# openMVG/openMVG

Measured on NVIDIA B200. Metric: BA LM-iters/sec, higher is better.
Workload: dtype f64

## Files before the change

openmvg_b200/csrc/ba.cu:

```cuda
#include "ba_kernels.cuh"
#include <cub/device/device_radix_sort.cuh>

#include <algorithm>
#include <cmath>
#include <cstring>
#include <limits>
#include <memory>
#include <chrono>
#include <vector>

using namespace omvg;
using namespace omvg::ba;

namespace {

enum Slot { S_COST = 0, S_MODEL, S_STEP2_PT, S_STEP2_POSE, S_STEP2_INTR, S_X2_PT, S_X2_POSE, S_X2_INTR,
            S_GMAX_PT, S_GMAX_CAM, S_GMAX_INTR, S_PCG_IT, S_PCG_RES, S_PCG_B, S_CAND_COST, S_COUNT = 16 };

int model_nparams(int m) {
  switch (m) { case 1: return 3; case 2: return 4; case 3: return 6; case 4: return 8; case 5: return 7; case OMVG_CAMERA_SPHERICAL: return 0; default: return -1; }
}
int model_ndata(int m) { return m == OMVG_CAMERA_SPHERICAL ? 2 : model_nparams(m); }

template <typename T> struct DevBuf {
// ... 17 lines not shown
  int ni8 = 0, nred = 0, words = 0, nnzb = 0, eval_blocks = 0, eval_grid = 0, kiu = KI, gj_grid = 0, ics_chunks = 64;
  std::vector<int> perm;
  DevBuf<int> d_perm;
  std::vector<int> h_intr_model;
  DevBuf<double> pose[2], intr[2], pt[2], pose0, intr0, pt0;
  DevBuf<int> intr_model, obs_pose, obs_intr, obs_pt, pt_start, cam_start, cam_obs;
  DevBuf<double> obs_xy;
  DevBuf<double> r, Jp, Jc, Ji, camR[2], camdR, camrec[2];
  DevBuf<double> sc_pt, sc_cam, sc_intr, diag_pt, diag_cam, diag_intr, lmD_pt, lmD_cam, lmD_intr, g_cam, g_intr;
  DevBuf<double> EtE, Etb, EtFi, FtF, FiFi, Einv, step_pt, step_red;
  DevBuf<unsigned char> pt_single;
  DevBuf<unsigned> bitmap, intr_mask; DevBuf<int> wprefix, rowptr, cols;
  DevBuf<double> Scc, Sci, Sii, rhs, Minv_c, Minv_i, work_i;
  DevBuf<double> z, res, pvec, w, zeta, pcg_part;
  DevBuf<double> gW, bX, bR, bP, bW, bZ, pcg2_part;
  DevBuf<int> agg_of, agg_start, agg_cams, brow, nb_start, nb_list; DevBuf<unsigned short> blk_lcol; int nb_max = 0;
  DevBuf<double> cE, cT, cCv, cYv, cCv2, cAW, bP2; int ng = 0, agg_maxsize = 0;
  DevBuf<double> dA, dT;
  DevBuf<double> part, part2, part3, icol_part, scal;
  DevBuf<int> fail;
  DevBuf<unsigned long long> pcg_tim;
  DevBuf<double> corner_rep;
  DevBuf<double> GE;
  DevBuf<double> obs_w; DevBuf<unsigned char> obs_flags, pt_fixed; DevBuf<unsigned> pt_mask;
  DevBuf<unsigned char> pt_gcp, pt_removed, pt_now; DevBuf<unsigned> rej_bits; DevBuf<unsigned long long> rej_cnt;
  bool reject_ready = false;
  int n_slow = 0;
  bool has_ext = false; int npri = 0; double prior_huber_a = 0; DevBuf<int> prior_pose; DevBuf<double> prior_center, prior_weight, rP, JP;
  double *h_scal = nullptr;
  cudaEvent_t ev0 = nullptr, ev1 = nullptr, evj0 = nullptr, evj1 = nullptr;
  long long launches = 0;
};

namespace {

#define LAUNCH_CHECK() OMVG_CUDA(cudaGetLastError())

struct PhaseTimer {
  bool on = getenv("OMVG_BA_TIMING") != nullptr; const char *what;
  std::chrono::steady_clock::time_point t0 = std::chrono::steady_clock::now();
  explicit PhaseTimer(const char *w) : what(w) {}
  void lap(const char *name) { if (!on) return; const auto t1 = std::chrono::steady_clock::now(); fprintf(stderr, "[omvg_ba timing] %s/%s %.3f ms\n", what, name, std::chrono::duration<double, std::milli>(t1 - t0).count()); t0 = t1; }
};

int validate(const omvg_ba_problem *P) {
  if (!P) return fail(OMVG_E_ARG, "null problem");
// ... 224 lines not shown
  { std::vector<int> nb_start(ng + 1, 0), nb_list; std::vector<unsigned short> lcol(c->nnzb, 0); std::vector<int> mark(c->nc, -1);
    c->nb_max = 0;
    for (int g = 0; g < ng; ++g) {
      const int first = (int)nb_list.size();
      for (int t = agg_start[g]; t < agg_start[g + 1]; ++t) { const int a = agg_cams[t];
        for (int e = hp[a]; e < hp[a + 1]; ++e) { const int b = hcols[e]; if (mark[b] < first) { mark[b] = (int)nb_list.size(); nb_list.push_back(b); } lcol[e] = (unsigned short)std::min(65535, mark[b] - first); } }
      nb_start[g + 1] = (int)nb_list.size(); c->nb_max = std::max(c->nb_max, nb_start[g + 1] - first);
    }
    if ((rc = upload(c->nb_start, nb_start.data(), ng + 1, c->stream))) return rc;
    if ((rc = upload(c->nb_list, nb_list.data(), nb_list.size(), c->stream))) return rc;
    if ((rc = upload(c->blk_lcol, lcol.data(), lcol.size(), c->stream))) return rc;
    OMVG_CUDA(cudaStreamSynchronize(c->stream)); }
  const size_t nco_max = (size_t)ng * MAXW;
  if ((rc = c->cE.alloc(nco_max * nco_max))) return rc;
  if ((rc = c->cT.alloc(3 * (size_t)GJ_B * nco_max))) return rc;
  if ((rc = c->cCv.alloc((size_t)MAXRHS * nco_max))) return rc;
  if ((rc = c->cYv.alloc((size_t)MAXRHS * nco_max))) return rc;
  if ((rc = c->cCv2.alloc((size_t)MAXRHS * nco_max + 1)) || (rc = c->cAW.alloc((size_t)MAXRHS * nco_max + 1))) return rc;
  if ((rc = c->bP2.alloc((size_t)MAXRHS * 6 * c->nc))) return rc;
  OMVG_CUDA(cudaStreamSynchronize(c->stream));
  return c->Scc.alloc((size_t)c->nnzb * 36);
}

}

extern "C" {

void omvg_trim_cache(void) {
  omvg::pool_trim();
  ResPool &rp = res_pool(); std::lock_guard<std::mutex> g(rp.mu);
  int cur = 0; cudaGetDevice(&cur);
  for (int d = 0; d < 16; ++d) { if (rp.free_[d].empty()) continue; cudaSetDevice(d);
    for (CtxRes &r : rp.free_[d]) { cudaFreeHost(r.h_scal); for (cudaEvent_t e : r.ev) cudaEventDestroy(e); cudaStreamDestroy(r.stream); cudaStreamDestroy(r.stream2); }
    rp.free_[d].clear(); }
  cudaSetDevice(cur);
}

void omvg_ba_default_options(omvg_ba_options *o) {
  if (!o) return;
  std::memset(o, 0, sizeof *o);
  o->intrinsics_opt = 14; o->extrinsics_opt = 6; o->structure_opt = 1; o->use_loss = 1; o->huber_a = 16.0;
  o->max_num_iterations = 50; o->max_consecutive_invalid_steps = 5;
  o->function_tolerance = 1e-6; o->gradient_tolerance = 1e-10; o->parameter_tolerance = 1e-8;
  o->initial_radius = 1e4; o->max_radius = 1e16; o->min_radius = 1e-32; o->min_relative_decrease = 1e-3;
  o->min_lm_diagonal = 1e-6; o->max_lm_diagonal = 1e32;
  o->pcg_tolerance = 1e-8; o->pcg_max_iterations = 2000; o->verbose = 0;
// ... 89 lines not shown
  for (int w = 0; w < 2; ++w) { AL(c->pose[w], 6 * c->nc); AL(c->intr[w], c->ni8); AL(c->pt[w], 3 * (size_t)c->np); AL(c->camR[w], 9 * c->nc); AL(c->camrec[w], (size_t)CAMREC * c->nc); }
  AL(c->camdR, 27 * c->nc);
  AL(c->r, 2 * no); AL(c->Jp, 6 * no); AL(c->Jc, 12 * no); AL(c->Ji, 2 * KI * no);
  AL(c->sc_pt, 3 * (size_t)c->np); AL(c->sc_cam, 6 * c->nc); AL(c->sc_intr, c->ni8);
  AL(c->diag_pt, 3 * (size_t)c->np); AL(c->diag_cam, 6 * c->nc); AL(c->diag_intr, c->ni8);
  AL(c->lmD_pt, 3 * (size_t)c->np); AL(c->lmD_cam, 6 * c->nc); AL(c->lmD_intr, c->ni8); AL(c->g_cam, 6 * c->nc); AL(c->g_intr, c->ni8);
  AL(c->EtFi, 3 * KI * (size_t)c->np); AL(c->FtF, 36 * (size_t)c->nc); AL(c->FiFi, 64 * (size_t)c->ni);
  AL(c->EtE, 6 * (size_t)c->np); AL(c->Etb, 3 * (size_t)c->np); AL(c->Einv, 9 * (size_t)c->np); AL(c->step_pt, 3 * (size_t)c->np); AL(c->step_red, c->nred);
  AL(c->intr_mask, c->ni);
  AL(c->Sci, (size_t)c->ni8 * 6 * c->nc); AL(c->Sii, (size_t)c->ni8 * c->ni8); AL(c->rhs, c->nred); AL(c->Minv_c, 36 * (size_t)c->nc); AL(c->Minv_i, (size_t)c->ni * KI * KI);
  AL(c->work_i, (size_t)c->ni8 * c->ni8 + c->ni8);
  AL(c->gW, (size_t)MAXW * 6 * c->nc);
  AL(c->bX, (size_t)MAXRHS * 6 * c->nc); AL(c->bR, (size_t)MAXRHS * 6 * c->nc); AL(c->bP, (size_t)MAXRHS * 6 * c->nc); AL(c->bW, (size_t)MAXRHS * 6 * c->nc); AL(c->bZ, (size_t)MAXRHS * 6 * c->nc);
  AL(c->pcg2_part, (size_t)c->n_sms * PCG2_V);
  AL(c->z, c->nred); AL(c->res, c->nred); AL(c->pvec, c->nred); AL(c->w, c->nred); AL(c->zeta, c->nred); AL(c->pcg_part, 3 * (size_t)c->n_sms * 2);
  if (c->npri) { AL(c->rP, 3 * c->npri); AL(c->JP, 18 * c->npri); }
  AL(c->part, std::max(c->eval_blocks, 1024) + 2); AL(c->part2, 1024); AL(c->part3, 1024); c->ics_chunks = (int)std::max<long long>(1, std::min<long long>(4ll * c->n_sms / std::max(1, c->ni), (c->no + 2047) / 2048));
  AL(c->icol_part, (size_t)c->ni * c->ics_chunks * ICS_W); AL(c->scal, S_COUNT); AL(c->fail, 1);
#undef AL
  OMVG_CUDA(cudaMemsetAsync(c->scal.p, 0, S_COUNT * sizeof(double), s));
  tm.lap("allocations");
  if ((rc = build_structure(c))) return rc;
  tm.lap("structure");
  OMVG_CUDA(cudaStreamWaitEvent(s, c->ev_up, 0));
  setup_gather_xy_kernel<<<(unsigned)((no + 255) / 256), 256, 0, s>>>(c->d_perm.p, reinterpret_cast<const double2 *>(raw_xy.p), raw_w.p, raw_fl.p, no,
                                                                  reinterpret_cast<double2 *>(c->obs_xy.p), c->obs_w.p, c->obs_flags.p); LAUNCH_CHECK();
  c->launches++;
  if ((rc = omvg_ba_reset(c))) return rc;
  OMVG_CUDA(cudaStreamSynchronize(s));
  guard.release();
  *out = c; return OMVG_OK;
}

int omvg_ba_reset(omvg_ba_ctx *c) {
  if (!c) return fail(OMVG_E_ARG, "null ctx");
  OMVG_CUDA(cudaSetDevice(c->device));
  OMVG_CUDA(cudaMemcpyAsync(c->pose[0].p, c->pose0.p, 6 * c->nc * sizeof(double), cudaMemcpyDeviceToDevice, c->stream));
  OMVG_CUDA(cudaMemcpyAsync(c->intr[0].p, c->intr0.p, c->ni8 * sizeof(double), cudaMemcpyDeviceToDevice, c->stream));
  if (c->np) OMVG_CUDA(cudaMemcpyAsync(c->pt[0].p, c->pt0.p, 3 * (size_t)c->np * sizeof(double), cudaMemcpyDeviceToDevice, c->stream));
  return OMVG_OK;
}

int omvg_ba_destroy(omvg_ba_ctx *c) {
  if (!c) return OMVG_OK;
  cudaSetDevice(c->device);
  if (c->stream) cudaStreamSynchronize(c->stream);
// ... 54 lines not shown
  double radius = O->initial_radius, decrease_factor = 2.0;
  int iteration = 0, n_success = 0, n_fail = 0, n_invalid = 0, termination = 3;
  double x_norm = -1.0;
  bool step_is_successful = true, failure = false;
  double reference_cost = x_cost, accumulated_reference = 0.0, current_cost = x_cost;
  long long pcg_total = 0;
  int coarse_age = -1; double last_pcg_its = 0, fresh_pcg_its = 1e30; bool fresh_pending = false;
  static const int coarse_every = getenv("OMVG_BA_COARSE_EVERY") ? std::max(1, atoi(getenv("OMVG_BA_COARSE_EVERY"))) : 3;
  if (!c->gj_grid) {
    int per_sm = 1; OMVG_CUDA(cudaOccupancyMaxActiveBlocksPerMultiprocessor(&per_sm, coarse_invert_kernel, 256, 0));
    c->gj_grid = c->n_sms * std::max(1, std::min(per_sm, 2));
  }

  for (;;) {
    if (step_is_successful) ++n_success; else ++n_fail;
    if (iteration >= O->max_num_iterations) { termination = 3; break; }
    if (step_is_successful && gmax <= O->gradient_tolerance) { termination = 2; break; }
    if (radius <= O->min_radius) { termination = 4; break; }
    ++iteration;
    { Diag3 DG{}; DG.s[0] = Diag3Seg{c->diag_pt.p, c->lmD_pt.p, 3 * c->np}; DG.s[1] = Diag3Seg{c->diag_cam.p, c->lmD_cam.p, 6 * c->nc}; DG.s[2] = Diag3Seg{c->diag_intr.p, c->lmD_intr.p, c->ni8};
      const int nb = std::max(1, std::min(2 * c->n_sms, (3 * c->np + 255) / 256));
      lm_diag3_kernel<<<dim3(nb, 3), 256, 0, c->stream>>>(DG, O->min_lm_diagonal, O->max_lm_diagonal, radius); LAUNCH_CHECK(); }
    if (m.pts_free && !c->corner_rep.p) { if ((rc = c->corner_rep.alloc((size_t)CORNER_REPS * (KI * KI + KI)))) return rc; }
    { Zero4 Z{}; Z.p[0] = c->Scc.p; Z.n[0] = (long long)c->nnzb * 36; Z.p[1] = c->Sci.p; Z.n[1] = (long long)c->Sci.n; Z.p[2] = c->Sii.p; Z.n[2] = (long long)c->Sii.n;
      Z.p[3] = m.pts_free ? c->corner_rep.p : c->rhs.p; Z.n[3] = m.pts_free ? (long long)c->corner_rep.n : 0;
      const int nb = (int)std::max<long long>(1, std::min<long long>(4 * c->n_sms, (Z.n[0] + 255) / 256));
      zero4_kernel<<<dim3(nb, 4), 256, 0, c->stream>>>(Z); LAUNCH_CHECK(); }
    SchurArgs SA{}; SA.r = c->r.p; SA.Jp = c->Jp.p; SA.Jc = c->Jc.p; SA.Ji = c->Ji.p; SA.EtE = c->EtE.p; SA.Etb = c->Etb.p; SA.EtFi = c->EtFi.p; SA.lmD_pt = c->lmD_pt.p; SA.pt_single = c->pt_single.p; SA.FtF = c->FtF.p; SA.FiFi = c->FiFi.p; SA.g_cam = c->g_cam.p; SA.g_intr = c->g_intr.p;
    SA.obs_pose = c->obs_pose.p; SA.obs_intr = c->obs_intr.p; SA.obs_pt = c->obs_pt.p; SA.pt_start = c->pt_start.p; SA.n = c->no; SA.n_poses = c->nc; SA.n_intr = c->ni;
    SA.pts_free = m.pts_free; SA.kiu = c->kiu; SA.bsr = Bsr{c->bitmap.p, c->wprefix.p, c->rowptr.p, c->words}; SA.Scc = c->Scc.p; SA.Sci = c->Sci.p; SA.Sii = c->Sii.p; SA.rhs = c->rhs.p;
    SA.Einv = c->Einv.p; SA.fail = c->fail.p;
    { const int ninit = std::max(std::max(36 * c->nc, 64 * c->ni), c->nred); s_init_kernel<<<(ninit + 255) / 256, 256, 0, c->stream>>>(SA); LAUNCH_CHECK(); }
    SA.n_points = c->np;
    if (m.pts_free) {
      if (!c->GE.p) { if ((rc = c->GE.alloc(36 * (size_t)c->no))) return rc; }
      { const unsigned sg = (unsigned)((c->no + SCHUR_THREADS - 1) / SCHUR_THREADS);
#define STAGE(K) schur_stage_kernel<K><<<sg, SCHUR_THREADS, 0, c->stream>>>(SA, c->GE.p, c->corner_rep.p)
        switch (c->kiu) {
          case 3: STAGE(3); break;
          case 4: STAGE(4); break;
          case 6: STAGE(6); break;
          case 7: STAGE(7); break;
          default: STAGE(8); break;
        }
#undef STAGE
      }
      LAUNCH_CHECK();
      corner_fold_kernel<<<1, 96, 0, c->stream>>>(c->corner_rep.p, c->obs_intr.p, c->nc, c->ni, c->Sii.p, c->rhs.p); LAUNCH_CHECK(); c->launches++;
      static const int occ2 = [] { int o = 1; cudaOccupancyMaxActiveBlocksPerMultiprocessor(&o, schur_pair_kernel, 256, 0); return std::max(1, o); }();
      schur_pair_kernel<<<c->n_sms * occ2, 256, 0, c->stream>>>(SA, c->GE.p); LAUNCH_CHECK(); c->launches += 2;
      SA.skip_fast = 1;
    }
    if (!m.pts_free || c->n_slow > 0) { schur_kernel<<<(unsigned)((c->no + SCHUR_THREADS - 1) / SCHUR_THREADS), SCHUR_THREADS, 0, c->stream>>>(SA); LAUNCH_CHECK(); }
    mirror_kernel<<<(c->nc * 32 + 255) / 256, 256, 0, c->stream>>>(c->Scc.p, SA.bsr, c->cols.p, c->nc); LAUNCH_CHECK();
    c->launches += 2;
    finish_cam_kernel<<<(c->nc + 63) / 64, 64, 0, c->stream>>>(c->Scc.p, SA.bsr, c->lmD_cam.p, m.pose_mask, c->nc, c->Minv_c.p, c->fail.p, use_dense ? 0 : 1); LAUNCH_CHECK();
    finish_intr_kernel<<<1, 256, 0, c->stream>>>(c->Sii.p, c->lmD_intr.p, c->intr_mask.p, c->ni8, c->Minv_i.p, c->work_i.p, c->fail.p, (use_pcg3 || use_dense) ? 0 : 1); LAUNCH_CHECK();
    PcgArgs PA{}; PA.Scc = c->Scc.p; PA.rowptr = c->rowptr.p; PA.cols = c->cols.p; PA.Sci = c->Sci.p; PA.Sii = c->Sii.p; PA.rhs = c->rhs.p; PA.Minv_c = c->Minv_c.p; PA.Minv_i = c->Minv_i.p;
    PA.n_poses = c->nc; PA.ni8 = c->ni8; PA.z = c->z.p; PA.res = c->res.p; PA.p = c->pvec.p; PA.w = c->w.p; PA.zeta = c->zeta.p; PA.part = c->pcg_part.p;
    PA.tol = O->pcg_tolerance; PA.max_iter = O->pcg_max_iterations; PA.out = c->scal.p + S_PCG_IT;
    const bool use_coarse = !use_dense && nw > 0 && c->nc >= 2;
    const Coarse CO{c->agg_of.p, c->agg_start.p, c->agg_cams.p, c->ng, nw, use_coarse ? c->ng * nw : 0};
    if (use_coarse) {
      const int nco = CO.nco;
      const bool refresh = nco > 0 && (coarse_age < 0 || coarse_age >= coarse_every || last_pcg_its > 1.5 * fresh_pcg_its + 5);
      if (refresh) { coarse_age = 0; fresh_pending = true; }
      ++coarse_age;
      if (refresh) {
        OMVG_CUDA(cudaMemsetAsync(c->cE.p, 0, (size_t)nco * nco * sizeof(double), c->stream));
        coarse_assemble_kernel<<<(c->nnzb + 127) / 128, 128, 0, c->stream>>>(c->Scc.p, c->brow.p, c->cols.p, c->nnzb, c->gW.p, c->nc, CO, c->cE.p); LAUNCH_CHECK();
        double *Ep = c->cE.p, *Tp = c->cT.p; int nn = nco; int *fp = c->fail.p;
        static const bool gj_timing = getenv("OMVG_BA_GJ_TIMING") != nullptr;
        unsigned long long *tp = nullptr;
        if (gj_timing) { if (!c->pcg_tim.p) { if ((rc = c->pcg_tim.alloc(8))) return rc; } OMVG_CUDA(cudaMemsetAsync(c->pcg_tim.p, 0, 64, c->stream)); tp = c->pcg_tim.p; }
        void *cargs[] = {&Ep, &nn, &Tp, &fp, &tp};
        const int mt = (nco + CT - 1) / CT;
        const int gj = std::max(1, std::min(c->gj_grid, mt * mt));
        OMVG_CUDA(cudaLaunchCooperativeKernel((void *)coarse_invert_kernel, dim3(gj), dim3(256), cargs, 0, c->stream));
// ... 335 lines not shown
```

openmvg_b200/csrc/ba_kernels.cuh:

```cuda
#pragma once
#include "common.cuh"
#include <cooperative_groups.h>
#include <cfloat>

namespace omvg { namespace ba {

namespace cg = cooperative_groups;
constexpr int KI = OMVG_BA_INTR_STRIDE;

template <int N> struct Dual { double a; double v[N]; };
template <int N> __device__ __forceinline__ Dual<N> dconst(double s) { Dual<N> d; d.a = s; for (int i = 0; i < N; ++i) d.v[i] = 0; return d; }
template <int N> __device__ __forceinline__ Dual<N> dvar(double s, int k) { Dual<N> d = dconst<N>(s); d.v[k] = 1.0; return d; }
template <int N> __device__ __forceinline__ Dual<N> operator+(const Dual<N> &f, const Dual<N> &g) { Dual<N> h; h.a = f.a + g.a; for (int i = 0; i < N; ++i) h.v[i] = f.v[i] + g.v[i]; return h; }
template <int N> __device__ __forceinline__ Dual<N> operator-(const Dual<N> &f, const Dual<N> &g) { Dual<N> h; h.a = f.a - g.a; for (int i = 0; i < N; ++i) h.v[i] = f.v[i] - g.v[i]; return h; }
template <int N> __device__ __forceinline__ Dual<N> operator*(const Dual<N> &f, const Dual<N> &g) { Dual<N> h; h.a = f.a * g.a; for (int i = 0; i < N; ++i) h.v[i] = f.a * g.v[i] + f.v[i] * g.a; return h; }
template <int N> __device__ __forceinline__ Dual<N> operator/(const Dual<N> &f, const Dual<N> &g) { Dual<N> h; const double gi = 1.0 / g.a, q = f.a * gi; h.a = q; for (int i = 0; i < N; ++i) h.v[i] = (f.v[i] - q * g.v[i]) * gi; return h; }
template <int N> __device__ __forceinline__ Dual<N> dsqrt(const Dual<N> &f) { Dual<N> h; h.a = sqrt(f.a); const double t = 1.0 / (2.0 * h.a); for (int i = 0; i < N; ++i) h.v[i] = t * f.v[i]; return h; }
template <int N> __device__ __forceinline__ Dual<N> dcos(const Dual<N> &f) { Dual<N> h; h.a = cos(f.a); const double s = -sin(f.a); for (int i = 0; i < N; ++i) h.v[i] = s * f.v[i]; return h; }
template <int N> __device__ __forceinline__ Dual<N> dsin(const Dual<N> &f) { Dual<N> h; h.a = sin(f.a); const double c = cos(f.a); for (int i = 0; i < N; ++i) h.v[i] = c * f.v[i]; return h; }

template <int THREADS> __device__ __forceinline__ double block_sum(double v, double *sh ) {
  #pragma unroll
  for (int o = 16; o > 0; o >>= 1) v += __shfl_down_sync(0xffffffffu, v, o);
  const int lane = threadIdx.x & 31, w = threadIdx.x >> 5;
// ... 532 lines not shown
}
__global__ void bitmap_mark_kernel(const int *__restrict__ obs_pose, const int *__restrict__ obs_pt, const int *__restrict__ pt_start,
                                   long long n, unsigned *__restrict__ bitmap, int words) {
  const long long o = (long long)blockIdx.x * blockDim.x + threadIdx.x; if (o >= n) return;
  const int a = obs_pose[o], j = obs_pt[o];
  for (long long u = pt_start[j]; u < pt_start[j + 1]; ++u) { const int b = obs_pose[u]; atomicOr(&bitmap[(size_t)a * words + (b >> 5)], 1u << (b & 31)); }
}
__global__ void bitmap_rowcount_kernel(const unsigned *__restrict__ bitmap, int nc, int words, int *__restrict__ wprefix, int *__restrict__ rowcount) {
  const int a = blockIdx.x * blockDim.x + threadIdx.x; if (a >= nc) return;
  int c = 0; for (int w = 0; w < words; ++w) { wprefix[(size_t)a * words + w] = c; c += __popc(bitmap[(size_t)a * words + w]); }
  rowcount[a] = c;
}
__global__ void bitmap_cols_kernel(const unsigned *__restrict__ bitmap, const int *__restrict__ rowptr, int nc, int words, int *__restrict__ cols) {
  const int a = blockIdx.x * blockDim.x + threadIdx.x; if (a >= nc) return;
  int k = rowptr[a];
  for (int w = 0; w < words; ++w) { unsigned m = bitmap[(size_t)a * words + w]; while (m) { const int b = __ffs(m) - 1; m &= m - 1; cols[k++] = w * 32 + b; } }
}

struct SchurArgs {
  const double *r, *Jp, *Jc, *Ji, *EtE, *Etb, *EtFi, *lmD_pt;
  const int *obs_pose, *obs_intr, *obs_pt, *pt_start; const unsigned char *pt_single;
  const double *FtF, *FiFi, *g_cam, *g_intr;
  long long n; int n_poses, n_intr, pts_free, kiu;
  int n_points;
  int skip_fast;
  Bsr bsr;
  double *Scc;
  double *Sci;
  double *Sii;
  double *rhs;
  double *Einv;
  int *fail;
};

__global__ void s_init_kernel(SchurArgs A) {
  const int i = blockIdx.x * blockDim.x + threadIdx.x;
  const int nc36 = 36 * A.n_poses, ni64 = 64 * A.n_intr, nred = 6 * A.n_poses + KI * A.n_intr;
  if (i < nc36) { const int p = i / 36; A.Scc[36 * (size_t)bsr_find(A.bsr, p, p) + i % 36] = A.FtF[i]; }
  if (i < ni64) { const int q = i / 64, e = i % 64; A.Sii[(size_t)(KI * q + e / KI) * (KI * A.n_intr) + KI * q + e % KI] = A.FiFi[i]; }
  if (i < nred) A.rhs[i] = i < 6 * A.n_poses ? A.g_cam[i] : A.g_intr[i - 6 * A.n_poses];
}

constexpr int SCHUR_THREADS = 128;
__global__ void __launch_bounds__(SCHUR_THREADS) schur_kernel(SchurArgs A) {
  __shared__ double s_ii[KI * KI + KI];
  __shared__ int s_q0;
  const long long t = (long long)blockIdx.x * SCHUR_THREADS + threadIdx.x;
  const long long n = A.n;
  if (threadIdx.x < KI * KI + KI) s_ii[threadIdx.x] = 0.0;
  if (threadIdx.x == 0) s_q0 = A.obs_intr[(long long)blockIdx.x * SCHUR_THREADS];
  __syncthreads();
  const int q0 = s_q0;
  const int nred_c = 6 * A.n_poses, ni8 = KI * A.n_intr;
  bool mine = t < n;
  if (mine && A.skip_fast && A.pts_free) { const int j = A.obs_pt[t]; mine = !(A.pt_single[j] != 0 && A.pt_start[j + 1] - A.pt_start[j] <= 32); }
  if (mine) {
    const int j = A.obs_pt[t], ct = A.obs_pose[t], qt = A.obs_intr[t];
    double jc[12], ji[2 * KI], jp[6];
    #pragma unroll
    for (int k = 0; k < 12; ++k) jc[k] = A.Jc[k * n + t];
    #pragma unroll
// ... 62 lines not shown
          const double e0 = jp[0] * ji[a] + jp[3] * ji[KI + a], e1 = jp[1] * ji[a] + jp[4] * ji[KI + a], e2 = jp[2] * ji[a] + jp[5] * ji[KI + a];
          gt_i[a] = inv[0] * e0 + inv[1] * e1 + inv[2] * e2; gt_i[KI + a] = inv[3] * e0 + inv[4] * e1 + inv[5] * e2; gt_i[2 * KI + a] = inv[6] * e0 + inv[7] * e1 + inv[8] * e2;
          const double rv = -(e0 * ie[0] + e1 * ie[1] + e2 * ie[2]);
          if (rv != 0.0) atomicAdd(&A.rhs[nred_c + KI * qt + a], rv);
          if (ji[a] == 0.0 && ji[KI + a] == 0.0) continue;
          #pragma unroll
          for (int b = 0; b < 6; ++b) atomicAdd(&sci_row0[(size_t)a * nred_c + b], ji[a] * jc[b] + ji[KI + a] * jc[6 + b]);
        }
      }
      for (long long u = A.pt_start[j]; u < A.pt_start[j + 1]; ++u) {
        const int cu = A.obs_pose[u];
        if (cu < ct && single) continue;
        double up[6], uc[12], efu[18];
        #pragma unroll
        for (int k = 0; k < 6; ++k) up[k] = A.Jp[k * n + u];
        #pragma unroll
        for (int k = 0; k < 12; ++k) uc[k] = A.Jc[k * n + u];
        #pragma unroll
        for (int a = 0; a < 3; ++a)
          #pragma unroll
          for (int c = 0; c < 6; ++c) efu[a * 6 + c] = up[a] * uc[c] + up[3 + a] * uc[6 + c];
        if (cu >= ct) {
          double *blk = A.Scc + 36 * (size_t)bsr_find(A.bsr, ct, cu);
          #pragma unroll
          for (int a = 0; a < 6; ++a)
            #pragma unroll
            for (int b = 0; b < 6; ++b) atomicAdd(&blk[a * 6 + b], -(gt_c[a] * efu[b] + gt_c[6 + a] * efu[6 + b] + gt_c[12 + a] * efu[12 + b]));
        }
        if (!single) {
          const int qu = A.obs_intr[u];
          #pragma unroll
          for (int a = 0; a < KI; ++a) {
            if (gt_i[a] == 0.0 && gt_i[KI + a] == 0.0 && gt_i[2 * KI + a] == 0.0) continue;
            #pragma unroll
            for (int b = 0; b < 6; ++b) atomicAdd(&A.Sci[(size_t)(KI * qt + a) * nred_c + 6 * cu + b], -(gt_i[a] * efu[b] + gt_i[KI + a] * efu[6 + b] + gt_i[2 * KI + a] * efu[12 + b]));
            #pragma unroll
            for (int b = 0; b < KI; ++b) {
              const double ui0 = b < A.kiu ? A.Ji[b * n + u] : 0.0, ui1 = b < A.kiu ? A.Ji[(KI + b) * n + u] : 0.0;
              const double e0 = up[0] * ui0 + up[3] * ui1, e1 = up[1] * ui0 + up[4] * ui1, e2 = up[2] * ui0 + up[5] * ui1;
              const double v = gt_i[a] * e0 + gt_i[KI + a] * e1 + gt_i[2 * KI + a] * e2;
              if (v != 0.0) atomicAdd(&A.Sii[(size_t)(KI * qt + a) * ni8 + KI * qu + b], -v);
            }
          }
        }
      }
    }
  }
  __syncthreads();
  if (threadIdx.x < KI * KI + KI) {
    const double v = s_ii[threadIdx.x];
// ... 76 lines not shown
      }
    }
  } else {
    #pragma unroll
    for (int k = 0; k < 36; ++k) gs[k] = 0.0;
  }
  __syncwarp();
  { const long long t0 = (long long)blockIdx.x * SCHUR_THREADS + 32 * warp;
    const long long nrec = n - t0 < 32 ? n - t0 : 32;
    if (nrec > 0) {
      double *dst = GE + 36 * (size_t)t0;
      #pragma unroll 4
      for (int e = lane; e < 36 * (int)nrec; e += 32) dst[e] = ge_s[warp][(e / 36) * GE_LD + e % 36];
    } }
}
__global__ void corner_fold_kernel(const double *__restrict__ corner_rep, const int *__restrict__ obs_intr, int n_poses, int n_intr, double *__restrict__ Sii, double *__restrict__ rhs) {
  const int e = threadIdx.x; if (e >= KI * KI + KI) return;
  const int q0 = obs_intr[0], ni8 = KI * n_intr;
  double v = 0; for (int rp2 = 0; rp2 < CORNER_REPS; ++rp2) v += corner_rep[(size_t)rp2 * (KI * KI + KI) + e];
  if (v == 0.0) return;
  if (e < KI * KI) atomicAdd(&Sii[(size_t)(KI * q0 + e / KI) * ni8 + KI * q0 + e % KI], v);
  else atomicAdd(&rhs[6 * n_poses + KI * q0 + (e - KI * KI)], v);
}
__global__ void __launch_bounds__(256) schur_pair_kernel(SchurArgs A, const double *__restrict__ GE) {
  const int lane = threadIdx.x & 31;
  const int gwarp = (blockIdx.x * blockDim.x + threadIdx.x) >> 5, nwarps = (gridDim.x * blockDim.x) >> 5;
  const int ea = lane / 6, eb2 = lane % 6, fa = (32 + lane) / 6, fb = (32 + lane) % 6;
  int t0n = 0, Kn = 0;
  if (gwarp < A.n_points) { t0n = A.pt_start[gwarp]; Kn = A.pt_start[gwarp + 1] - t0n; }
  { const char *pf = reinterpret_cast<const char *>(GE + 36 * (size_t)t0n) + 128 * lane;
    if (128 * lane < 288 * Kn) asm volatile("prefetch.global.L1 [%0];" :: "l"(pf)); if (128 * (lane + 32) < 288 * Kn) asm volatile("prefetch.global.L1 [%0];" :: "l"(pf + 4096)); }
  for (int j = gwarp; j < A.n_points; j += nwarps) {
    const int t0 = t0n, K = Kn;
    if (j + nwarps < A.n_points) {
      t0n = A.pt_start[j + nwarps]; Kn = A.pt_start[j + nwarps + 1] - t0n;
      const char *pf = reinterpret_cast<const char *>(GE + 36 * (size_t)t0n) + 128 * lane;
      if (128 * lane < 288 * Kn) asm volatile("prefetch.global.L1 [%0];" :: "l"(pf)); if (128 * (lane + 32) < 288 * Kn && Kn <= 32) asm volatile("prefetch.global.L1 [%0];" :: "l"(pf + 4096));
    }
    if (K == 0 || K > 32 || !A.pt_single[j]) continue;
    const int cam_l = lane < K ? A.obs_pose[t0 + lane] : 0;
    const unsigned lowmask = (1u << (cam_l & 31)) - 1u;
    int rp = 0, wp = 0; unsigned bm = 0;
    { const int c0 = __shfl_sync(0xffffffffu, cam_l, 0); const size_t w = (size_t)c0 * A.bsr.words + (cam_l >> 5); rp = A.bsr.rowptr[c0]; wp = A.bsr.wprefix[w]; bm = A.bsr.bitmap[w]; }
    const double *ge = GE + 36 * (size_t)t0;
    for (int tt = 0; tt < K; ++tt) {
      const int ctt = __shfl_sync(0xffffffffu, cam_l, tt);
      const int cur = (lane < K && cam_l >= ctt) ? rp + wp + __popc(bm & lowmask) : -1;
      if (tt + 1 < K) { const int cn = __shfl_sync(0xffffffffu, cam_l, tt + 1); const size_t w = (size_t)cn * A.bsr.words + (cam_l >> 5); rp = A.bsr.rowptr[cn]; wp = A.bsr.wprefix[w]; bm = A.bsr.bitmap[w]; }
      const double *gt = ge + 36 * tt;
      const double g0 = gt[ea], g1 = gt[6 + ea], g2 = gt[12 + ea];
      const double h0 = lane < 4 ? gt[fa] : 0.0, h1 = lane < 4 ? gt[6 + fa] : 0.0, h2 = lane < 4 ? gt[12 + fa] : 0.0;
      unsigned todo = __ballot_sync(0xffffffffu, cur >= 0);
      while (todo) {
        const int u = __ffs(todo) - 1; todo &= todo - 1;
        const int bi = __shfl_sync(0xffffffffu, cur, u);
        double *blk = A.Scc + 36 * (size_t)bi;
        const double *ef = ge + 36 * u + 18;
        atomicAdd(blk + lane, -(g0 * ef[eb2] + g1 * ef[6 + eb2] + g2 * ef[12 + eb2]));
        if (lane < 4) atomicAdd(blk + 32 + lane, -(h0 * ef[fb] + h1 * ef[6 + fb] + h2 * ef[12 + fb]));
      }
    }
  }
}

__global__ void mirror_kernel(double *__restrict__ Scc, Bsr B, const int *__restrict__ cols, int n_poses) {
  const int a = (blockIdx.x * blockDim.x + threadIdx.x) >> 5, lane = threadIdx.x & 31;
  if (a >= n_poses) return;
  for (int e = B.rowptr[a]; e < B.rowptr[a + 1]; ++e) {
    const int b = cols[e]; if (b >= a) break;
    const double *src = Scc + 36 * (size_t)bsr_find(B, b, a); double *dst = Scc + 36 * (size_t)e;
    for (int k = lane; k < 36; k += 32) dst[k] = src[(k % 6) * 6 + k / 6];
  }
}

__global__ void finish_cam_kernel(double *__restrict__ Scc, Bsr B, const double *__restrict__ lmD_cam, unsigned pose_mask, int n_poses,
                                  double *__restrict__ Minv, int *__restrict__ fail, int need_inverse) {
  const int p = blockIdx.x * blockDim.x + threadIdx.x; if (p >= n_poses) return;
  double *blk = Scc + 36 * (size_t)bsr_find(B, p, p);
  double M[36];
  for (int k = 0; k < 6; ++k) { if ((pose_mask >> k) & 1) blk[k * 6 + k] += lmD_cam[6 * p + k] * lmD_cam[6 * p + k]; else blk[k * 6 + k] = 1.0; }
  if (!need_inverse) return;
  for (int k = 0; k < 36; ++k) M[k] = blk[k];
  for (int k = 0; k < 6; ++k) {
    double d = M[k * 6 + k]; for (int q = 0; q < k; ++q) d -= M[k * 6 + q] * M[k * 6 + q];
    if (!(d > 0.0) || !isfinite(d)) { atomicExch(fail, 2); return; }
    d = sqrt(d); M[k * 6 + k] = d;
    for (int i = k + 1; i < 6; ++i) { double s = M[i * 6 + k]; for (int q = 0; q < k; ++q) s -= M[i * 6 + q] * M[k * 6 + q]; M[i * 6 + k] = s / d; }
  }
  for (int c = 0; c < 6; ++c) {
    double b[6]; for (int i = 0; i < 6; ++i) b[i] = i == c ? 1.0 : 0.0;
    for (int i = 0; i < 6; ++i) { double s = b[i]; for (int q = 0; q < i; ++q) s -= M[i * 6 + q] * b[q]; b[i] = s / M[i * 6 + i]; }
    for (int i = 5; i >= 0; --i) { double s = b[i]; for (int q = i + 1; q < 6; ++q) s -= M[q * 6 + i] * b[q]; b[i] = s / M[i * 6 + i]; }
    for (int i = 0; i < 6; ++i) Minv[36 * (size_t)p + i * 6 + c] = b[i];
  }
}
// ... 1251 lines not shown
```

Measured before the change: 414.2.

## Replace atomic Schur pair scatter with presorted per-block gather and drop mirror pass

Precomputes at setup a list of observation pairs sorted by target upper-triangular camera block. Each iteration then uses one warp per block to accumulate that block in registers, butterfly-reduce it, and write it directly along with its transpose. This removes the per-point atomicAdd scatter into Scc, the separate mirror kernel and the zeroing of Scc. The slow path now also writes transposed blocks atomically. The cost is extra device memory for the pair list, heavier setup, and possible load imbalance when a few blocks own many pairs.

```diff
diff --git a/openmvg_b200/csrc/ba.cu b/openmvg_b200/csrc/ba.cu
--- a/openmvg_b200/csrc/ba.cu
+++ b/openmvg_b200/csrc/ba.cu
@@ -1,5 +1,6 @@
 #include "ba_kernels.cuh"
 #include <cub/device/device_radix_sort.cuh>
+#include <cub/device/device_scan.cuh>
 
 #include <algorithm>
 #include <cmath>
@@ -63,6 +64,7 @@
   DevBuf<unsigned long long> pcg_tim;
   DevBuf<double> corner_rep;
   DevBuf<double> GE;
+  DevBuf<unsigned long long> pairs; DevBuf<int> gstart, gblk, gblkT; int nwork = 0;
   DevBuf<double> obs_w; DevBuf<unsigned char> obs_flags, pt_fixed; DevBuf<unsigned> pt_mask;
   DevBuf<unsigned char> pt_gcp, pt_removed, pt_now; DevBuf<unsigned> rej_bits; DevBuf<unsigned long long> rej_cnt;
   bool reject_ready = false;
@@ -333,6 +335,55 @@
   return c->Scc.alloc((size_t)c->nnzb * 36);
 }
 
+int build_pair_lists(omvg_ba_ctx *c) {
+  int rc;
+  std::vector<int> hp(c->nc + 1), hcols(c->nnzb);
+  OMVG_CUDA(cudaMemcpyAsync(hp.data(), c->rowptr.p, (c->nc + 1) * sizeof(int), cudaMemcpyDeviceToHost, c->stream));
+  OMVG_CUDA(cudaMemcpyAsync(hcols.data(), c->cols.p, (size_t)c->nnzb * sizeof(int), cudaMemcpyDeviceToHost, c->stream));
+  OMVG_CUDA(cudaStreamSynchronize(c->stream));
+  auto find = [&](int a, int b) { return (int)(std::lower_bound(hcols.begin() + hp[a], hcols.begin() + hp[a + 1], b) - hcols.begin()); };
+  std::vector<int> wpos(c->nnzb, -1), gblk, gblkT;
+  for (int a = 0; a < c->nc; ++a) { const int e = find(a, a); wpos[e] = (int)gblk.size(); gblk.push_back(e); gblkT.push_back(e); }
+  for (int a = 0; a < c->nc; ++a)
+    for (int e = hp[a]; e < hp[a + 1]; ++e) if (hcols[e] > a) { wpos[e] = (int)gblk.size(); gblk.push_back(e); gblkT.push_back(find(hcols[e], a)); }
+  c->nwork = (int)gblk.size();
+  cudaStream_t s = c->stream;
+  DevBuf<int> d_wpos;
+  if ((rc = upload(c->gblk, gblk.data(), gblk.size(), s)) || (rc = upload(c->gblkT, gblkT.data(), gblkT.size(), s)) || (rc = upload(d_wpos, wpos.data(), wpos.size(), s))) return rc;
+  DevBuf<long long> cnt, offs; DevBuf<unsigned char> tmp;
+  if ((rc = cnt.alloc(c->np + 1)) || (rc = offs.alloc(c->np + 1)) || (rc = c->gstart.alloc(c->nwork + 1))) return rc;
+  pair_count_kernel<<<(c->np + 256) / 256, 256, 0, s>>>(c->pt_start.p, c->pt_single.p, c->obs_pose.p, c->np, cnt.p); LAUNCH_CHECK();
+  size_t tb = 0;
+  OMVG_CUDA(cub::DeviceScan::ExclusiveSum(nullptr, tb, cnt.p, offs.p, c->np + 1, s));
+  if ((rc = tmp.alloc(tb))) return rc;
+  OMVG_CUDA(cub::DeviceScan::ExclusiveSum(tmp.p, tb, cnt.p, offs.p, c->np + 1, s));
+  long long total = 0;
+  OMVG_CUDA(cudaMemcpyAsync(&total, offs.p + c->np, sizeof total, cudaMemcpyDeviceToHost, s));
+  OMVG_CUDA(cudaStreamSynchronize(s));
+  if (total > std::numeric_limits<int>::max()) return fail(OMVG_E_UNSUPPORTED, "%lld camera-pair terms of the Schur complement (at most 2^31 - 1)", total);
+  const int n = (int)total;
+  if (n > 0) {
+    DevBuf<int> k0, k1; DevBuf<unsigned long long> p0;
+    if ((rc = k0.alloc(n)) || (rc = k1.alloc(n)) || (rc = p0.alloc(n)) || (rc = c->pairs.alloc(n))) return rc;
+    pair_fill_kernel<<<(c->np + 255) / 256, 256, 0, s>>>(c->pt_start.p, c->pt_single.p, c->obs_pose.p, c->np, offs.p, Bsr{c->bitmap.p, c->wprefix.p, c->rowptr.p, c->words}, d_wpos.p, k0.p, p0.p); LAUNCH_CHECK();
+    int kbits = 1; while ((1ll << kbits) < c->nwork) ++kbits;
+    size_t sb = 0;
+    OMVG_CUDA(cub::DeviceRadixSort::SortPairs(nullptr, sb, k0.p, k1.p, p0.p, c->pairs.p, n, 0, kbits, s));
+    if (sb > tmp.n && (rc = tmp.alloc(sb))) return rc;
+    sb = tmp.n;
+    OMVG_CUDA(cub::DeviceRadixSort::SortPairs(tmp.p, sb, k0.p, k1.p, p0.p, c->pairs.p, n, 0, kbits, s));
+    setup_starts_kernel<<<(unsigned)((n + 256) / 256), 256, 0, s>>>(k1.p, n, c->nwork, c->gstart.p); LAUNCH_CHECK();
+    OMVG_CUDA(cudaStreamSynchronize(s));
+    c->launches += 2;
+  } else {
+    OMVG_CUDA(cudaMemsetAsync(c->gstart.p, 0, (c->nwork + 1) * sizeof(int), s));
+    OMVG_CUDA(cudaStreamSynchronize(s));
+  }
+  c->launches += 1;
+  if (getenv("OMVG_BA_TIMING")) fprintf(stderr, "[omvg_ba structure] %d upper S blocks, %d pair-list entries (%.1f MB)\n", c->nwork, n, n * 8e-6);
+  return OMVG_OK;
+}
+
 }
 
 extern "C" {
@@ -468,6 +519,8 @@
   tm.lap("allocations");
   if ((rc = build_structure(c))) return rc;
   tm.lap("structure");
+  if ((rc = build_pair_lists(c))) return rc;
+  tm.lap("pair lists");
   OMVG_CUDA(cudaStreamWaitEvent(s, c->ev_up, 0));
   setup_gather_xy_kernel<<<(unsigned)((no + 255) / 256), 256, 0, s>>>(c->d_perm.p, reinterpret_cast<const double2 *>(raw_xy.p), raw_w.p, raw_fl.p, no,
                                                                   reinterpret_cast<double2 *>(c->obs_xy.p), c->obs_w.p, c->obs_flags.p); LAUNCH_CHECK();
@@ -568,16 +621,17 @@
       const int nb = std::max(1, std::min(2 * c->n_sms, (3 * c->np + 255) / 256));
       lm_diag3_kernel<<<dim3(nb, 3), 256, 0, c->stream>>>(DG, O->min_lm_diagonal, O->max_lm_diagonal, radius); LAUNCH_CHECK(); }
     if (m.pts_free && !c->corner_rep.p) { if ((rc = c->corner_rep.alloc((size_t)CORNER_REPS * (KI * KI + KI)))) return rc; }
-    { Zero4 Z{}; Z.p[0] = c->Scc.p; Z.n[0] = (long long)c->nnzb * 36; Z.p[1] = c->Sci.p; Z.n[1] = (long long)c->Sci.n; Z.p[2] = c->Sii.p; Z.n[2] = (long long)c->Sii.n;
+    { Zero4 Z{}; Z.p[0] = c->Scc.p; Z.n[0] = m.pts_free ? 0 : (long long)c->nnzb * 36;
+      Z.p[1] = c->Sci.p; Z.n[1] = (long long)c->Sci.n; Z.p[2] = c->Sii.p; Z.n[2] = (long long)c->Sii.n;
       Z.p[3] = m.pts_free ? c->corner_rep.p : c->rhs.p; Z.n[3] = m.pts_free ? (long long)c->corner_rep.n : 0;
-      const int nb = (int)std::max<long long>(1, std::min<long long>(4 * c->n_sms, (Z.n[0] + 255) / 256));
+      const long long zmax = std::max(std::max(Z.n[0], Z.n[1]), std::max(Z.n[2], Z.n[3]));
+      const int nb = (int)std::max<long long>(1, std::min<long long>(4 * c->n_sms, (zmax + 255) / 256));
       zero4_kernel<<<dim3(nb, 4), 256, 0, c->stream>>>(Z); LAUNCH_CHECK(); }
     SchurArgs SA{}; SA.r = c->r.p; SA.Jp = c->Jp.p; SA.Jc = c->Jc.p; SA.Ji = c->Ji.p; SA.EtE = c->EtE.p; SA.Etb = c->Etb.p; SA.EtFi = c->EtFi.p; SA.lmD_pt = c->lmD_pt.p; SA.pt_single = c->pt_single.p; SA.FtF = c->FtF.p; SA.FiFi = c->FiFi.p; SA.g_cam = c->g_cam.p; SA.g_intr = c->g_intr.p;
     SA.obs_pose = c->obs_pose.p; SA.obs_intr = c->obs_intr.p; SA.obs_pt = c->obs_pt.p; SA.pt_start = c->pt_start.p; SA.n = c->no; SA.n_poses = c->nc; SA.n_intr = c->ni;
     SA.pts_free = m.pts_free; SA.kiu = c->kiu; SA.bsr = Bsr{c->bitmap.p, c->wprefix.p, c->rowptr.p, c->words}; SA.Scc = c->Scc.p; SA.Sci = c->Sci.p; SA.Sii = c->Sii.p; SA.rhs = c->rhs.p;
     SA.Einv = c->Einv.p; SA.fail = c->fail.p;
     { const int ninit = std::max(std::max(36 * c->nc, 64 * c->ni), c->nred); s_init_kernel<<<(ninit + 255) / 256, 256, 0, c->stream>>>(SA); LAUNCH_CHECK(); }
-    SA.n_points = c->np;
     if (m.pts_free) {
       if (!c->GE.p) { if ((rc = c->GE.alloc(36 * (size_t)c->no))) return rc; }
       { const unsigned sg = (unsigned)((c->no + SCHUR_THREADS - 1) / SCHUR_THREADS);
@@ -593,13 +647,13 @@
       }
       LAUNCH_CHECK();
       corner_fold_kernel<<<1, 96, 0, c->stream>>>(c->corner_rep.p, c->obs_intr.p, c->nc, c->ni, c->Sii.p, c->rhs.p); LAUNCH_CHECK(); c->launches++;
-      static const int occ2 = [] { int o = 1; cudaOccupancyMaxActiveBlocksPerMultiprocessor(&o, schur_pair_kernel, 256, 0); return std::max(1, o); }();
-      schur_pair_kernel<<<c->n_sms * occ2, 256, 0, c->stream>>>(SA, c->GE.p); LAUNCH_CHECK(); c->launches += 2;
+      schur_gather_kernel<<<(unsigned)(((long long)c->nwork * 32 + GATHER_THREADS - 1) / GATHER_THREADS), GATHER_THREADS, 0, c->stream>>>(
+          c->GE.p, c->gstart.p, reinterpret_cast<const int2 *>(c->pairs.p), c->gblk.p, c->gblkT.p, c->nwork, c->brow.p, c->FtF.p, c->Scc.p); LAUNCH_CHECK();
+      c->launches += 2;
       SA.skip_fast = 1;
     }
     if (!m.pts_free || c->n_slow > 0) { schur_kernel<<<(unsigned)((c->no + SCHUR_THREADS - 1) / SCHUR_THREADS), SCHUR_THREADS, 0, c->stream>>>(SA); LAUNCH_CHECK(); }
-    mirror_kernel<<<(c->nc * 32 + 255) / 256, 256, 0, c->stream>>>(c->Scc.p, SA.bsr, c->cols.p, c->nc); LAUNCH_CHECK();
-    c->launches += 2;
+    c->launches += 1;
     finish_cam_kernel<<<(c->nc + 63) / 64, 64, 0, c->stream>>>(c->Scc.p, SA.bsr, c->lmD_cam.p, m.pose_mask, c->nc, c->Minv_c.p, c->fail.p, use_dense ? 0 : 1); LAUNCH_CHECK();
     finish_intr_kernel<<<1, 256, 0, c->stream>>>(c->Sii.p, c->lmD_intr.p, c->intr_mask.p, c->ni8, c->Minv_i.p, c->work_i.p, c->fail.p, (use_pcg3 || use_dense) ? 0 : 1); LAUNCH_CHECK();
     PcgArgs PA{}; PA.Scc = c->Scc.p; PA.rowptr = c->rowptr.p; PA.cols = c->cols.p; PA.Sci = c->Sci.p; PA.Sii = c->Sii.p; PA.rhs = c->rhs.p; PA.Minv_c = c->Minv_c.p; PA.Minv_i = c->Minv_i.p;
diff --git a/openmvg_b200/csrc/ba_kernels.cuh b/openmvg_b200/csrc/ba_kernels.cuh
--- a/openmvg_b200/csrc/ba_kernels.cuh
+++ b/openmvg_b200/csrc/ba_kernels.cuh
@@ -578,7 +578,6 @@
   const int *obs_pose, *obs_intr, *obs_pt, *pt_start; const unsigned char *pt_single;
   const double *FtF, *FiFi, *g_cam, *g_intr;
   long long n; int n_poses, n_intr, pts_free, kiu;
-  int n_points;
   int skip_fast;
   Bsr bsr;
   double *Scc;
@@ -592,7 +591,7 @@
 __global__ void s_init_kernel(SchurArgs A) {
   const int i = blockIdx.x * blockDim.x + threadIdx.x;
   const int nc36 = 36 * A.n_poses, ni64 = 64 * A.n_intr, nred = 6 * A.n_poses + KI * A.n_intr;
-  if (i < nc36) { const int p = i / 36; A.Scc[36 * (size_t)bsr_find(A.bsr, p, p) + i % 36] = A.FtF[i]; }
+  if (i < nc36 && !A.pts_free) { const int p = i / 36; A.Scc[36 * (size_t)bsr_find(A.bsr, p, p) + i % 36] = A.FtF[i]; }
   if (i < ni64) { const int q = i / 64, e = i % 64; A.Sii[(size_t)(KI * q + e / KI) * (KI * A.n_intr) + KI * q + e % KI] = A.FiFi[i]; }
   if (i < nred) A.rhs[i] = i < 6 * A.n_poses ? A.g_cam[i] : A.g_intr[i - 6 * A.n_poses];
 }
@@ -701,10 +700,15 @@
           for (int c = 0; c < 6; ++c) efu[a * 6 + c] = up[a] * uc[c] + up[3 + a] * uc[6 + c];
         if (cu >= ct) {
           double *blk = A.Scc + 36 * (size_t)bsr_find(A.bsr, ct, cu);
+          double *blt = cu > ct ? A.Scc + 36 * (size_t)bsr_find(A.bsr, cu, ct) : nullptr;
           #pragma unroll
           for (int a = 0; a < 6; ++a)
             #pragma unroll
-            for (int b = 0; b < 6; ++b) atomicAdd(&blk[a * 6 + b], -(gt_c[a] * efu[b] + gt_c[6 + a] * efu[6 + b] + gt_c[12 + a] * efu[12 + b]));
+            for (int b = 0; b < 6; ++b) {
+              const double v = -(gt_c[a] * efu[b] + gt_c[6 + a] * efu[6 + b] + gt_c[12 + a] * efu[12 + b]);
+              atomicAdd(&blk[a * 6 + b], v);
+              if (blt) atomicAdd(&blt[b * 6 + a], v);
+            }
         }
         if (!single) {
           const int qu = A.obs_intr[u];
@@ -827,55 +831,85 @@
   if (e < KI * KI) atomicAdd(&Sii[(size_t)(KI * q0 + e / KI) * ni8 + KI * q0 + e % KI], v);
   else atomicAdd(&rhs[6 * n_poses + KI * q0 + (e - KI * KI)], v);
 }
-__global__ void __launch_bounds__(256) schur_pair_kernel(SchurArgs A, const double *__restrict__ GE) {
-  const int lane = threadIdx.x & 31;
-  const int gwarp = (blockIdx.x * blockDim.x + threadIdx.x) >> 5, nwarps = (gridDim.x * blockDim.x) >> 5;
-  const int ea = lane / 6, eb2 = lane % 6, fa = (32 + lane) / 6, fb = (32 + lane) % 6;
-  int t0n = 0, Kn = 0;
-  if (gwarp < A.n_points) { t0n = A.pt_start[gwarp]; Kn = A.pt_start[gwarp + 1] - t0n; }
-  { const char *pf = reinterpret_cast<const char *>(GE + 36 * (size_t)t0n) + 128 * lane;
-    if (128 * lane < 288 * Kn) asm volatile("prefetch.global.L1 [%0];" :: "l"(pf)); if (128 * (lane + 32) < 288 * Kn) asm volatile("prefetch.global.L1 [%0];" :: "l"(pf + 4096)); }
-  for (int j = gwarp; j < A.n_points; j += nwarps) {
-    const int t0 = t0n, K = Kn;
-    if (j + nwarps < A.n_points) {
-      t0n = A.pt_start[j + nwarps]; Kn = A.pt_start[j + nwarps + 1] - t0n;
-      const char *pf = reinterpret_cast<const char *>(GE + 36 * (size_t)t0n) + 128 * lane;
-      if (128 * lane < 288 * Kn) asm volatile("prefetch.global.L1 [%0];" :: "l"(pf)); if (128 * (lane + 32) < 288 * Kn && Kn <= 32) asm volatile("prefetch.global.L1 [%0];" :: "l"(pf + 4096));
-    }
-    if (K == 0 || K > 32 || !A.pt_single[j]) continue;
-    const int cam_l = lane < K ? A.obs_pose[t0 + lane] : 0;
-    const unsigned lowmask = (1u << (cam_l & 31)) - 1u;
-    int rp = 0, wp = 0; unsigned bm = 0;
-    { const int c0 = __shfl_sync(0xffffffffu, cam_l, 0); const size_t w = (size_t)c0 * A.bsr.words + (cam_l >> 5); rp = A.bsr.rowptr[c0]; wp = A.bsr.wprefix[w]; bm = A.bsr.bitmap[w]; }
-    const double *ge = GE + 36 * (size_t)t0;
-    for (int tt = 0; tt < K; ++tt) {
-      const int ctt = __shfl_sync(0xffffffffu, cam_l, tt);
-      const int cur = (lane < K && cam_l >= ctt) ? rp + wp + __popc(bm & lowmask) : -1;
-      if (tt + 1 < K) { const int cn = __shfl_sync(0xffffffffu, cam_l, tt + 1); const size_t w = (size_t)cn * A.bsr.words + (cam_l >> 5); rp = A.bsr.rowptr[cn]; wp = A.bsr.wprefix[w]; bm = A.bsr.bitmap[w]; }
-      const double *gt = ge + 36 * tt;
-      const double g0 = gt[ea], g1 = gt[6 + ea], g2 = gt[12 + ea];
-      const double h0 = lane < 4 ? gt[fa] : 0.0, h1 = lane < 4 ? gt[6 + fa] : 0.0, h2 = lane < 4 ? gt[12 + fa] : 0.0;
-      unsigned todo = __ballot_sync(0xffffffffu, cur >= 0);
-      while (todo) {
-        const int u = __ffs(todo) - 1; todo &= todo - 1;
-        const int bi = __shfl_sync(0xffffffffu, cur, u);
-        double *blk = A.Scc + 36 * (size_t)bi;
-        const double *ef = ge + 36 * u + 18;
-        atomicAdd(blk + lane, -(g0 * ef[eb2] + g1 * ef[6 + eb2] + g2 * ef[12 + eb2]));
-        if (lane < 4) atomicAdd(blk + 32 + lane, -(h0 * ef[fb] + h1 * ef[6 + fb] + h2 * ef[12 + fb]));
-      }
-    }
-  }
-}
-
-__global__ void mirror_kernel(double *__restrict__ Scc, Bsr B, const int *__restrict__ cols, int n_poses) {
-  const int a = (blockIdx.x * blockDim.x + threadIdx.x) >> 5, lane = threadIdx.x & 31;
-  if (a >= n_poses) return;
-  for (int e = B.rowptr[a]; e < B.rowptr[a + 1]; ++e) {
-    const int b = cols[e]; if (b >= a) break;
-    const double *src = Scc + 36 * (size_t)bsr_find(B, b, a); double *dst = Scc + 36 * (size_t)e;
-    for (int k = lane; k < 36; k += 32) dst[k] = src[(k % 6) * 6 + k / 6];
-  }
+__device__ __forceinline__ bool pair_fast(const int *__restrict__ pt_start, const unsigned char *__restrict__ pt_single, int j, int &t0, int &K) {
+  t0 = pt_start[j]; K = pt_start[j + 1] - t0;
+  return pt_single[j] != 0 && K >= 1 && K <= 32;
+}
+__global__ void pair_count_kernel(const int *__restrict__ pt_start, const unsigned char *__restrict__ pt_single, const int *__restrict__ obs_pose,
+                                  int n_points, long long *__restrict__ count) {
+  const int j = blockIdx.x * blockDim.x + threadIdx.x; if (j > n_points) return;
+  long long cnt = 0; int t0, K;
+  if (j < n_points && pair_fast(pt_start, pt_single, j, t0, K))
+    for (int t = 0; t < K; ++t) { const int ct = obs_pose[t0 + t]; for (int u = 0; u < K; ++u) cnt += obs_pose[t0 + u] >= ct; }
+  count[j] = cnt;
+}
+__global__ void pair_fill_kernel(const int *__restrict__ pt_start, const unsigned char *__restrict__ pt_single, const int *__restrict__ obs_pose,
+                                 int n_points, const long long *__restrict__ offs, Bsr B, const int *__restrict__ wpos,
+                                 int *__restrict__ key, unsigned long long *__restrict__ pair) {
+  const int j = blockIdx.x * blockDim.x + threadIdx.x; if (j >= n_points) return;
+  int t0, K; if (!pair_fast(pt_start, pt_single, j, t0, K)) return;
+  long long o = offs[j];
+  for (int t = 0; t < K; ++t) {
+    const int ct = obs_pose[t0 + t];
+    for (int u = 0; u < K; ++u) {
+      const int cu = obs_pose[t0 + u]; if (cu < ct) continue;
+      key[o] = wpos[bsr_find(B, ct, cu)];
+      pair[o] = ((unsigned long long)(unsigned)(t0 + u) << 32) | (unsigned)(t0 + t);
+      ++o;
+    }
+  }
+}
+
+constexpr int GATHER_THREADS = 128;
+__global__ void __launch_bounds__(GATHER_THREADS) schur_gather_kernel(const double *__restrict__ GE, const int *__restrict__ gstart, const int2 *__restrict__ pairs,
+                                                                      const int *__restrict__ gblk, const int *__restrict__ gblkT, int nwork,
+                                                                      const int *__restrict__ brow, const double *__restrict__ FtF, double *__restrict__ Scc) {
+  const int w = (int)(((long long)blockIdx.x * GATHER_THREADS + threadIdx.x) >> 5), lane = threadIdx.x & 31;
+  if (w >= nwork) return;
+  double acc[36];
+  #pragma unroll
+  for (int i = 0; i < 36; ++i) acc[i] = 0.0;
+  const int e1 = gstart[w + 1];
+  for (int e = gstart[w] + lane; e < e1; e += 32) {
+    const int2 pr = pairs[e];
+    const double2 *g2 = reinterpret_cast<const double2 *>(GE + 36 * (size_t)pr.x);
+    const double2 *f2 = reinterpret_cast<const double2 *>(GE + 36 * (size_t)pr.y + 18);
+    double g[18], f[18];
+    #pragma unroll
+    for (int k = 0; k < 9; ++k) { const double2 v = g2[k]; g[2 * k] = v.x; g[2 * k + 1] = v.y; }
+    #pragma unroll
+    for (int k = 0; k < 9; ++k) { const double2 v = f2[k]; f[2 * k] = v.x; f[2 * k + 1] = v.y; }
+    #pragma unroll
+    for (int a = 0; a < 3; ++a)
+      #pragma unroll
+      for (int r = 0; r < 6; ++r)
+        #pragma unroll
+        for (int c = 0; c < 6; ++c) acc[r * 6 + c] = fma(g[a * 6 + r], f[a * 6 + c], acc[r * 6 + c]);
+  }
+  double h[18], v[9];
+  { const bool up = lane & 16;
+    #pragma unroll
+    for (int i = 0; i < 18; ++i) { const double keep = up ? acc[18 + i] : acc[i], send = up ? acc[i] : acc[18 + i]; h[i] = keep + __shfl_xor_sync(0xffffffffu, send, 16); } }
+  { const bool up = lane & 8;
+    #pragma unroll
+    for (int i = 0; i < 9; ++i) { const double keep = up ? h[9 + i] : h[i], send = up ? h[i] : h[9 + i]; v[i] = keep + __shfl_xor_sync(0xffffffffu, send, 8); } }
+  #pragma unroll
+  for (int m = 4; m >= 1; m >>= 1)
+    #pragma unroll
+    for (int i = 0; i < 9; ++i) v[i] += __shfl_xor_sync(0xffffffffu, v[i], m);
+  const int s = lane & 7, q = lane >> 3;
+  double x = v[0];
+  #pragma unroll
+  for (int i = 1; i < 8; ++i) if (s == i) x = v[i];
+  const int eu = gblk[w], el = gblkT[w];
+  const double *ftf = FtF + 36 * (size_t)brow[eu];
+  auto put = [&](int idx, double sum) {
+    if (eu == el) { Scc[36 * (size_t)eu + idx] = ftf[idx] - sum; return; }
+    Scc[36 * (size_t)eu + idx] = -sum;
+    Scc[36 * (size_t)el + (idx % 6) * 6 + idx / 6] = -sum;
+  };
+  put(9 * q + s, x);
+  if (s == 0) put(9 * q + 8, v[8]);
 }
 
 __global__ void finish_cam_kernel(double *__restrict__ Scc, Bsr B, const double *__restrict__ lmD_cam, unsigned pose_mask, int n_poses,
```

Result: faster. 435.5, median of 6 (+5.1%).
